# lueelu/DistributedFFT

Measured on AMD Instinct MI355X. Metric: GFlops/s forward 3D C2C (5 N log2 N), 512^3 fp64, higher is better.
Workload: dtype f64; 1 GPU; 512x512x512 C2C fp64 forward, slab decomposition over 1 GPU(s), fused pipeline, input resident in HBM; parallelism=slab1, exchange=none (P=1)

## Files before the change

### distributedfft_amd/csrc/dfft_core.cpp

```cpp
#include <cmath>
#include <map>
#include <mutex>

#include "dfft_plan_impl.h"
#include "dfft_r2r.h"
#include "dfft_real.h"
#include "dfft_real_cols.h"

namespace dfft {

static thread_local std::string g_last_error;
void set_error(const std::string& msg) { g_last_error = msg; }
int  fail(int code, const std::string& msg) {
    g_last_error = msg;
    trace_on_error(code, msg);
    return code;
}
const std::string& last_error() { return g_last_error; }

struct TwKey {
    int  dev, n, dtype;
    bool operator<(const TwKey& o) const {
        if (dev != o.dev) return dev < o.dev;
        if (n != o.n) return n < o.n;
// ... 129 lines not shown
    if (!valid_dtype(dtype) || kind < DFFT_R2R_DCT2 || kind > DFFT_R2R_DST3 || n < 1 || s < 1) return 0;
    return r2r_fused_env() && r2r_fused(n, s, dtype, kind, vec != 0);
}
int dfft_conv_fused_applies(int dtype, long long n0, long long rows, long long ncols, long long plane, long long pitch, int rot, const void* in,
                            const void* out) {
    if (!valid_dtype(dtype) || n0 < 1 || n0 > 4096 || rows < 1 || ncols < 1 || plane < 1 || pitch < 1 || rot < 0) return 0;
    ConvLaunch L;
    std::memset(&L, 0, sizeof(L));
    L.dtype = dtype;
    L.n0 = (int)n0;
    L.rows = rows;
    L.ncols = ncols;
    L.plane = plane;
    L.pitch = pitch;
    L.rot = rot;
    L.in = in;
    L.out = const_cast<void*>(out);
    return conv_fused_applies(L) ? 1 : 0;
}

int dfft_cols_extent_supported(long long n, long long width, int dtype, int pairs) {
    if (n < 1 || width < 1 || !valid_dtype(dtype) || length_kind(n) == 0 || length_kind(n) == 3) return 0;
    return cols_extent_ok(n, width, dtype, pairs != 0, pairs != 0) ? 1 : 0;
}
int dfft_fft1d_any_extent_supported(long long n, long long s, int dtype, int in16, int out16) {
    if (n < 1 || s < 1 || !valid_dtype(dtype) || length_kind(n) == 0) return 0;
    return any_extent_ok(n, s, dtype, in16 != 0, out16 != 0) ? 1 : 0;
}

static void scratch_tables(BluesteinTables* T, long long n, int dtype, int dir) {
    T->n = n;
    T->M = bluestein_padded_length(n);
    T->dtype = dtype;
    T->dir = dir;
}
unsigned long long dfft_fft1d_any_scratch_bytes(long long n, long long s, long long batch, int dtype) {
    const int kind = length_kind(n);
    if (!valid_dtype(dtype) || s < 1 || batch < 1 || kind < 2) return 0;
    if (kind == 2) return (unsigned long long)batch * n * s * elem_bytes(dtype);
    if (!bluestein_extent_ok(n, s, dtype)) return 0;
    BluesteinTables T;
    scratch_tables(&T, n, dtype, DFFT_FORWARD);
    return bluestein_scratch_bytes(T, s, batch, bluestein_fused_env());
}
unsigned long long dfft_rfft1d_strided_scratch_bytes(long long n, long long s, long long batch, int dtype) {
    const int kind = length_kind(n);
// ... 175 lines not shown
```

### distributedfft_amd/csrc/dfft_fft_impl.h

```cpp
#pragma once
#include <atomic>
#include <cstdio>
#include <cstdlib>
#include <mutex>
#include <type_traits>

#include "dfft_butterfly.h"
#include "dfft_kernels.h"

namespace dfft {

template <int N_, int E_, int... Rs> struct Plan {
    static constexpr int N = N_, E = E_, T = N_ / E_, S = sizeof...(Rs);
    static constexpr int R[sizeof...(Rs)] = {Rs...};
    static_assert((Rs * ... * 1) == N_, "radix product must equal N");
    static_assert(((E_ % Rs == 0) && ...), "every radix must divide E");
    static_assert(N_ % E_ == 0, "E must divide N");
};

struct TuneDefault {
    static constexpr bool TWPOW = true;
    static constexpr bool OSTAGE = false;
    static constexpr bool NTL = false;
    static constexpr bool NTS = false;
// ... 17 lines not shown
    static constexpr bool OSTAGE = true;
    static constexpr bool NTL = true;
    static constexpr bool NTS = true;
    static constexpr int MIN_WAVES = 0;
    static constexpr int CB_OVERRIDE = 0;
    static constexpr bool PLAIN = false;
    static constexpr bool PREFETCH = true;
    static constexpr bool FULL_PREFETCH = false;
    static constexpr bool PLAIN_IN = false;
    static constexpr bool EARLY_WAIT = false;
    static constexpr bool ROT = false;
    static constexpr int ROT_IN = 0, ROT_OUT = 0;
};
struct TuneTransposedStoreFull : TuneTransposedStore {
    static constexpr bool FULL_PREFETCH = true;
    static constexpr bool PLAIN_IN = true;
};
struct TuneTransposedStoreFullEarly : TuneTransposedStoreFull {
    static constexpr bool EARLY_WAIT = true;
};
struct TuneTransposedStoreEarly : TuneTransposedStore {
    static constexpr bool EARLY_WAIT = true;
};

struct TuneCols : TuneDefault {
    static constexpr bool PREFETCH = true;
};

template <class Base> struct Plain : Base {
    static constexpr bool PLAIN = true;
};

template <class Base> struct TransposedSide : Base {
    static constexpr bool NO_OWNED = true;
};
template <class T, class = void> struct tune_no_owned : std::false_type {};
template <class T> struct tune_no_owned<T, std::void_t<decltype(T::NO_OWNED)>> : std::bool_constant<T::NO_OWNED> {};

struct TuneStreamIn : TuneDefault {
    static constexpr bool NTL = true;
};
struct TuneColsStreamIn : TuneCols {
    static constexpr bool NTL = true;
};
struct TuneColsStreamOut : TuneCols {
    static constexpr bool NTS = true;
// ... 344 lines not shown
inline long long axis_max_offset(const AxisMap& m, int n) {
    long long mx = 0;
    const int nb = m.blk > 0 ? (n + m.blk - 1) / m.blk : 1;
    for (int ib = 0; ib < nb; ++ib) {
        const long long bt = m.sub > 1 ? (long long)(ib / m.sub) * m.blk_stride + (long long)(ib % m.sub) * m.sub_stride : (long long)ib * m.blk_stride;
        const int       cnt = (ib + 1) * m.blk <= n ? m.blk : n - ib * m.blk;
        const long long o = bt + (long long)(cnt - 1) * m.stride;
        if (o > mx) mx = o;
    }
    return mx;
}
inline bool tile_offsets_fit32(const FftLaunch& L) {
    auto fits = [&](const AxisMap& m) {
        const long long c = m.cstride < 0 ? -m.cstride : m.cstride;
        return axis_max_offset(m, L.n) + (kTileColsMax - 1) * c < (1ll << 32);
    };
    return fits(L.imap) && fits(L.omap);
}
template <class V, class P, int CB, int G, int DIR, bool GENERAL, class Tune>
__global__ void __attribute__((amdgpu_flat_work_group_size(1, KernelGeom<V, P, CB, G, Tune>::THREADS),
                               amdgpu_waves_per_eu(Tune::MIN_WAVES > 0 ? Tune::MIN_WAVES : 1)))
fft_tiles_kernel(const typename VecTraits<V>::G* in, typename VecTraits<V>::G* out,
                 const typename VecTraits<V>::W* __restrict__ tw, AxisMap imap, AxisMap omap, TileMap itile, TileMap otile,
                 unsigned ntiles, unsigned tiles_per_a, int ncols, unsigned a_first, double scale, RotMap rm) {
    using KG = KernelGeom<V, P, CB, G, Tune>;
    using VT = VecTraits<V>;
    using W = typename VT::W;
    using GV = typename VT::G;
    constexpr int E = P::E, T = P::T, GT = KG::GT, N = P::N, LANES = VT::LANES;
    extern __shared__ __attribute__((aligned(16))) char dfft_smem[];
    W* ldstw = reinterpret_cast<W*>(dfft_smem);
    V* lds = reinterpret_cast<V*>(dfft_smem + KG::TW_BYTES) + (threadIdx.x / GT) * KG::LDS_ELEMS;

    const int g = threadIdx.x / GT;
    const int tid = threadIdx.x - g * GT;
    const int c = tid % CB;
    const int j = tile_j<CB, KG::NW>(tid);

    constexpr int TWN = KG::TWMODE == TW_REG ? KG::TWN : 0;
    W twreg[TWN > 0 ? TWN : 1];
    const W* twr = stage_twiddles<V, P, DIR, KG, Tune::TWPOW>(twreg, ldstw, tw, j);
    constexpr bool TWPOW = Tune::TWPOW && KG::TWMODE == TW_REG;

    constexpr bool PLAIN = Tune::PLAIN && !GENERAL && !KG::OSTAGE && !Tune::ROT;
    constexpr bool PLAIN_IN = PLAIN || (Tune::PLAIN_IN && !GENERAL);
    constexpr int NREL = PLAIN ? 1 : E;
    constexpr int ON = N / LANES;
// ... 65 lines not shown
#pragma unroll
            for (int k = K0; k < K1; ++k) {
                long long off = PLAIN_IN ? (long long)(ir0 + (unsigned)k * istep) : (long long)irel[PLAIN_IN ? 0 : k];
                if (GENERAL) off += ((ilast >> k) & 1u) ? (long long)a * imap.last_delta : 0ll;
                if constexpr (Tune::ROT_IN == 2) off += (long long)(((cb0 + rj + k * rot_t) & rm.mask) - cb0);
                dst[k - K0] = VT::from_g(gload<Tune::NTL>(ip + off));
            }
        } else {
#pragma unroll
            for (int k = K0; k < K1; ++k) dst[k - K0] = VT::zero();
        }
    };
    auto load_tile = [&](unsigned t, V* dst) { load_part(t, dst, std::integral_constant<int, 0>{}, std::integral_constant<int, E>{}); };
    constexpr bool EARLY = Tune::EARLY_WAIT;
    constexpr bool P768 = P::N == 768 && E == 12 && sizeof(V) == 16;
    constexpr bool PREFETCH = Tune::PREFETCH && (E * (int)sizeof(V) / 4 <= kPrefetchMaxRegs || Tune::FULL_PREFETCH || P768) && KG::THREADS <= 512;
    constexpr int PF = PREFETCH ? E : (Tune::PREFETCH && KG::OSTAGE && E == 16 && sizeof(V) == 16 && KG::THREADS <= 512 && KG::PH == 1 ? E / 2 : 0);
    constexpr bool PARTIAL = PF > 0 && PF < E;
    using K0 = std::integral_constant<int, 0>;
    using KP = std::integral_constant<int, PF>;
    using KE = std::integral_constant<int, E>;
    V v[E];
    V vnext[PF > 0 ? PF : 1];
    if constexpr (PREFETCH) {
        if (blockIdx.x * G < ntiles) load_tile(blockIdx.x * G, v);
    } else if constexpr (PARTIAL) {
        if (blockIdx.x * G < ntiles) load_part(blockIdx.x * G, v, K0{}, KP{});
    }
    for (unsigned t0 = blockIdx.x * G; t0 < ntiles; t0 += tstep) {
        const unsigned tile = map_tile(t0 + g);
        bool valid = tile < ntiles;
        const unsigned al = tile / tiles_per_a;
        const unsigned b = tile - al * tiles_per_a;
        const unsigned a = al + a_first;
        if (GENERAL) valid = valid && ((int)(b * CB) + c < ncols);
        int ob0 = (int)(b * CB);
        if constexpr (Tune::ROT_OUT == 1) ob0 = (ob0 + rm.rot * (int)(a + (unsigned)rm.a0)) & rm.mask;
        GV* op = out + (long long)a * otile.a_stride + (long long)ob0 * otile.b_stride;

        if constexpr (PREFETCH) {
            if (t0 + tstep < ntiles) load_tile(t0 + tstep, vnext);
        } else if constexpr (PARTIAL) {
            load_part(t0, v + PF, KP{}, KE{});
            if (t0 + tstep < ntiles) load_part(t0 + tstep, vnext, K0{}, KP{});
        } else {
            load_tile(t0, v);
        }

        constexpr bool LOCALX = KG::LOCALX && !(GENERAL && P::N == 729 && CB > 1);
        run_stages<V, P, 0, DIR, CB, KG::PAD, KG::WAVE_LOCAL, KG::TWMODE, TWPOW, KG::PH, 1, KG::NW, LOCALX>(v, twr, lds, j, c);

        const typename real_of<W>::type sc = (typename real_of<W>::type)scale;

        if constexpr (KG::OSTAGE) {
            static_assert(!GENERAL || !KG::OSTAGE, "the staged store is a fast-path variant");
            constexpr int ROW = N + KG::OPAD;
            W* img = reinterpret_cast<W*>(lds);
            if constexpr (KG::PH == 1) {
                group_sync<KG::WAVE_LOCAL>();
#pragma unroll
                for (int k = 0; k < E; ++k)
#pragma unroll
                    for (int l = 0; l < LANES; ++l) img[(c * LANES + l) * ROW + j + T * k] = VT::lane(cscale(v[k], sc), l);
                group_sync<KG::WAVE_LOCAL>();
                if constexpr (EARLY && PF > 0) {
#pragma unroll
                    for (int k = 0; k < PF; ++k) pin_loaded(vnext[k]);
                }
                if (valid) {
#pragma unroll
                    for (int k = 0; k < E; ++k) {
                        const int lin = tid + GT * k;
                        const GV r = *reinterpret_cast<const GV*>(img + (lin / ON) * ROW + (lin % ON) * LANES);
                        gstore<Tune::NTS>(op + ostage_off(k), r);
                    }
                }
            } else {
                constexpr int CH = CB / KG::PH, EPH = E / KG::PH;
                const int     mine = c / CH, cl = c - mine * CH;
#pragma unroll
                for (int ph = 0; ph < KG::PH; ++ph) {
                    __syncthreads();
                    if (mine == ph) {
#pragma unroll
                        for (int k = 0; k < E; ++k)
#pragma unroll
                            for (int l = 0; l < LANES; ++l) img[(cl * LANES + l) * ROW + j + T * k] = VT::lane(cscale(v[k], sc), l);
// ... 7 lines not shown
                            gstore<Tune::NTS>(op + ostage_off(ph * EPH + k), r);
                        }
                    }
                }
            }
        } else if (valid) {
            if constexpr (EARLY && PF > 0) {
#pragma unroll
                for (int k = 0; k < PF; ++k) pin_loaded(vnext[k]);
            }
            unsigned or0 = orel[0];
            if constexpr (PLAIN) asm volatile("" : "+v"(or0));
#pragma unroll
            for (int k = 0; k < E; ++k) {
                long long off = PLAIN ? (long long)(or0 + (unsigned)k * ostep) : (long long)orel[PLAIN ? 0 : k];
                if (GENERAL) off += ((olast >> k) & 1u) ? (long long)a * omap.last_delta : 0ll;
                if constexpr (Tune::ROT_OUT == 2) off += (long long)(((ob0 + rot_j + k * rot_t) & rm.mask) - ob0);
                gstore<Tune::NTS>(op + off, VT::to_g(cscale(v[k], sc)));
            }
        }
        if constexpr (PF > 0) {
#pragma unroll
            for (int k = 0; k < PF; ++k) v[k] = vnext[k];
        }
    }
}

template <class V, class P, int CB> struct DualGeom {
    using W = typename VecTraits<V>::W;
    static constexpr int    LANES = VecTraits<V>::LANES, OPAD = LANES == 2 ? 2 : 1;
    static constexpr size_t BUDGET = 160 * 1024;
    static constexpr size_t TW_BYTES = ((size_t)P::N * sizeof(W) + 15) / 16 * 16;
    static constexpr bool   PADROW = (size_t)(P::N + OPAD) * CB * sizeof(V) + TW_BYTES <= BUDGET;
    static constexpr int    ROW = PADROW ? P::N + OPAD : P::N;
    static constexpr size_t LDS_BYTES = TW_BYTES + (size_t)ROW * CB * sizeof(V);
    static_assert(LDS_BYTES <= BUDGET, "dual tiles: tile + twiddle table must fit the workgroup's share of the CU's LDS");
};
template <class V, class P, int CB, int DIR, bool NT, bool ROT = false>
__global__ void __attribute__((amdgpu_flat_work_group_size(1, CB * P::T), amdgpu_waves_per_eu(1)))
fft_dual_tiles_kernel(const typename VecTraits<V>::G* in, typename VecTraits<V>::G* out, const typename VecTraits<V>::W* __restrict__ tw,
                      AxisMap imap, AxisMap omap, TileMap itile, TileMap otile, unsigned ntiles, unsigned tiles_per_a, unsigned a_first,
                      double scale, RotMap rm) {
    using VT = VecTraits<V>;
    using W = typename VT::W;
    using GV = typename VT::G;
    constexpr int E = P::E, T = P::T, GT = CB * T, N = P::N, LANES = VT::LANES;
// ... 399 lines not shown
    if (occ < 1) occ = 1;
    cache[dev].store(occ, std::memory_order_release);
    return occ;
}

inline long long persistent_grid(int cus, int blocks_per_cu, long long units, long long grid_limit = 0, int blocks_per_cu_limit = 0) {
    if (blocks_per_cu_limit > 0 && blocks_per_cu_limit < blocks_per_cu) blocks_per_cu = blocks_per_cu_limit;
    long long grid = (long long)cus * blocks_per_cu;
    if (grid_limit > 0 && grid > grid_limit) grid = grid_limit;
    return grid < units ? grid : units;
}

template <class V, class P, int CB, int G, int DIR, bool GENERAL, class Tune = TuneDefault>
hipError_t launch_variant(const FftLaunch& L, hipStream_t stream, int* blocks_per_cu_out = nullptr) {
    using KG = KernelGeom<V, P, CB, G, Tune>;
    auto kern = fft_tiles_kernel<V, P, CB, G, DIR, GENERAL, Tune>;
    static std::atomic<int> blocks_per_cu[kMaxDevices];
    hipError_t e;
    const int  bpc = resident_blocks_per_cu(reinterpret_cast<const void*>(kern), KG::THREADS, KG::LDS_BYTES, blocks_per_cu, &e);
    if (bpc == 0) return e;
    if (blocks_per_cu_out) *blocks_per_cu_out = bpc;
    const long long grid = persistent_grid(device_info().cus, bpc, (L.ntiles + G - 1) / G, L.grid_limit, L.blocks_per_cu_limit);
    if (grid < 1) return hipSuccess;
    (void)hipGetLastError();
    using GV = typename VecTraits<V>::G;
    hipLaunchKernelGGL(kern, dim3((unsigned)grid), dim3(KG::THREADS), KG::LDS_BYTES, stream, (const GV*)L.in, (GV*)L.out,
                       (const typename VecTraits<V>::W*)L.tw, L.imap, L.omap, L.itile, L.otile, (unsigned)L.ntiles,
                       (unsigned)L.tiles_per_a, L.ncols, (unsigned)L.a_first, L.scale == 0.0 ? 1.0 : L.scale, L.rot);
    e = hipGetLastError();
    if (e != hipSuccess) return launch_debug(e, "kernel launch", (int)KG::LDS_BYTES, KG::THREADS);
    return hipSuccess;
}

template <class V, class P, int CB, int DIR, bool NT, bool ROT = false> hipError_t launch_dual(const FftLaunch& L, hipStream_t stream) {
    using VT = VecTraits<V>;
    using W = typename VT::W;
    using GV = typename VT::G;
    constexpr size_t LDS_BYTES = DualGeom<V, P, CB>::LDS_BYTES;
    auto kern = fft_dual_tiles_kernel<V, P, CB, DIR, NT, ROT>;
    static std::atomic<int> attr_set[kMaxDevices];
    hipError_t e;
    if (resident_blocks_per_cu(reinterpret_cast<const void*>(kern), CB * P::T, LDS_BYTES, attr_set, &e, false) == 0) return e;
    const long long tiles_per_a = L.ncols / (2 * CB), ntiles = L.na * tiles_per_a;
    if (ntiles <= 0) return hipSuccess;
    if (ntiles >= (1ll << 31)) return hipErrorInvalidValue;
    const long long grid = persistent_grid(device_info().cus, 1, ntiles, L.grid_limit);
    (void)hipGetLastError();
    hipLaunchKernelGGL(kern, dim3((unsigned)grid), dim3(CB * P::T), LDS_BYTES, stream, (const GV*)L.in, (GV*)L.out, (const W*)L.tw, L.imap,
                       L.omap, L.itile, L.otile, (unsigned)ntiles, (unsigned)tiles_per_a, (unsigned)L.a_first, L.scale == 0.0 ? 1.0 : L.scale, L.rot);
    e = hipGetLastError();
    if (e != hipSuccess) return launch_debug(e, "kernel launch", (int)LDS_BYTES, CB * P::T);
    return hipSuccess;
}
// ... 139 lines not shown
        return launch_plan<V, P, PH, CBC / 2>(Lin, stream);
    } else if constexpr (CBC * P::T <= 1024) {
        if constexpr (CBO == 0 && can_tload<V, P>()) {
            if (tload_applies<V, P>(L)) {
                if (rot) return L.dir > 0 ? launch_tload<V, P, CBC, +1, true>(L, stream) : launch_tload<V, P, CBC, -1, true>(L, stream);
                return L.dir > 0 ? launch_tload<V, P, CBC, +1, false>(L, stream) : launch_tload<V, P, CBC, -1, false>(L, stream);
            }
        }
        if constexpr (VecTraits<V>::LANES == 2) {
            if (L.imap.nblk == 1 && L.imap.stride == 1 && L.imap.cstride != 1 && !(L.omap.nblk == 1 && L.omap.stride == 1 && L.omap.cstride != 1))
                return hipErrorInvalidValue;
        }
        using TT = TuneTransposedStore;
        using TTF = TuneTransposedStoreFull;
        constexpr bool can_stage = can_stage_store<V, P, CBO>();
        const bool staged = can_stage && !general && L.omap.nblk == 1 && L.omap.stride == 1 && L.omap.cstride != 1;
        constexpr bool can_full = can_stage && P::E == 16 && sizeof(V) == 16 && CBC * (int)sizeof(V) == 128 && CBC * P::T * GC <= 512;
        using TTFE = TuneTransposedStoreFullEarly;
        using TTE = TuneTransposedStoreEarly;
        const bool single_in = L.imap.nblk == 1 && L.imap.sub <= 1 && L.imap.last_delta == 0;
        const bool want_early = (L.hints & FFT_HINT_EARLY_WAIT) != 0;
        const int  full = (can_full && staged && L.dir > 0 && single_in && !(L.hints & FFT_HINT_HALF_PREFETCH)) ? (want_early ? 2 : 1) : 0;
        constexpr bool can_early = can_stage && P::N == 512 && sizeof(V) == 16;
        const bool early = can_early && staged && L.dir > 0 && want_early;
        constexpr bool can_dual = P::S > 1 && sizeof(V) == 16 && 2 * CBC * sizeof(V) == 128 && (P::N & (P::N - 1)) == 0 && (P::N / VecTraits<V>::LANES) % (CBC * P::T) == 0 &&
                                  (size_t)P::N * CBC * sizeof(V) + (size_t)P::N * sizeof(typename VecTraits<V>::W) <= 160 * 1024;
        if constexpr (!std::is_void<PH>::value && ((VecTraits<V>::LANES == 2 && P::N >= 2048) || (P::N == 1024 && VecTraits<V>::LANES == 1))) {
            static const bool x_dif2 = [] {
                const char* e = getenv("DFFT_X_DIF2");
                return !(e && *e == '0');
            }();
            constexpr int CBF = 128 / (int)sizeof(V);
            const bool    transposed = L.omap.nblk == 1 && L.omap.stride == 1 && L.omap.cstride != 1 && L.omap.last_delta == 0;
            constexpr bool want = P::N >= 2048 || VecTraits<V>::LANES == 1;
            if (x_dif2 && want && L.dir > 0 && !general && transposed && L.imap.cstride == 1 && L.itile.b_stride == 1 && L.imap.nblk == 1 && L.imap.sub <= 1 && L.ncols % CBF == 0 &&
                L.imap.last_delta == 0 && (axis_max_offset(L.imap, P::N / 2) + L.ncols) * (long long)sizeof(V) < (1ll << 32) && L.itile.b_stride == 1 &&
                (!rot || (L.rot.in_mode == 2 && L.rot.out_mode == 0))) {
                if (rot) return launch_dif2<V, PH, CBF, +1, true, true, false, false, 2, true>(L, stream);
                return launch_dif2<V, PH, CBF, +1, true, true, false, false, 0, true>(L, stream);
            }
        }
        if constexpr (can_dual) {
            static const bool no_dual = [] {
                const char* e = getenv("DFFT_NO_DUAL");
                return e && *e && *e != '0';
            }();
            const bool transposed = L.omap.nblk == 1 && L.omap.stride == 1 && L.omap.cstride != 1;
// ... 79 lines not shown
                return launch_variant<V, P, CBC, GC, -1, false, Plain<TuneCols>>(L, stream);
            }
        }
        const bool tr_side = !(L.imap.cstride == 1 && L.itile.b_stride == 1) || (!(L.omap.cstride == 1 && L.otile.b_stride == 1) && !(can_stage && staged));
        using TSCols = std::conditional_t<(KernelGeom<V, P, CBC, GC, TuneCols>::NW > 0), TransposedSide<TuneCols>, TuneCols>;
        using TSColsIn = std::conditional_t<(KernelGeom<V, P, CBC, GC, TuneColsStreamIn>::NW > 0), TransposedSide<TuneColsStreamIn>, TuneColsStreamIn>;
        using TSColsOut = std::conditional_t<(KernelGeom<V, P, CBC, GC, TuneColsStreamOut>::NW > 0), TransposedSide<TuneColsStreamOut>, TuneColsStreamOut>;
        if (tr_side) {
            if (L.dir > 0) {
                if (general) return launch_variant<V, P, CBC, GC, +1, true, TSCols>(L, stream);
                if (L.hints & FFT_HINT_STREAM_OUT) return launch_variant<V, P, CBC, GC, +1, false, TSColsOut>(L, stream);
                return launch_variant<V, P, CBC, GC, +1, false, TSCols>(L, stream);
            }
            if (general) return launch_variant<V, P, CBC, GC, -1, true, TSCols>(L, stream);
            if (L.hints & FFT_HINT_STREAM_IN) return launch_variant<V, P, CBC, GC, -1, false, TSColsIn>(L, stream);
            return launch_variant<V, P, CBC, GC, -1, false, TSCols>(L, stream);
        }
        if (L.dir > 0) {
            if (general) return launch_variant<V, P, CBC, GC, +1, true, TuneCols>(L, stream);
            if constexpr (can_full) {
                if (full == 2) return launch_variant<V, P, CBC, GC, +1, false, TTFE>(L, stream);
                if (full == 1) return launch_variant<V, P, CBC, GC, +1, false, TTF>(L, stream);
            }
            if constexpr (can_early)
                if (early) return launch_variant<V, P, CBC, GC, +1, false, TTE>(L, stream);
            if constexpr (can_stage)
                if (staged) return launch_variant<V, P, CBC, GC, +1, false, TT>(L, stream);
            if (L.hints & FFT_HINT_STREAM_OUT) return launch_variant<V, P, CBC, GC, +1, false, TuneColsStreamOut>(L, stream);
            return launch_variant<V, P, CBC, GC, +1, false, TuneCols>(L, stream);
        }
        if (general) return launch_variant<V, P, CBC, GC, -1, true, TuneCols>(L, stream);
        if constexpr (can_stage)
            if (staged) return launch_variant<V, P, CBC, GC, -1, false, TT>(L, stream);
        if (L.hints & FFT_HINT_STREAM_IN) return launch_variant<V, P, CBC, GC, -1, false, TuneColsStreamIn>(L, stream);
        return launch_variant<V, P, CBC, GC, -1, false, TuneCols>(L, stream);
    } else {
        return hipErrorInvalidValue;
    }
}

template <class P> bool make_pair_launch(const FftLaunch& L, FftLaunch& out) {
    static const bool disabled = [] {
        const char* e = getenv("DFFT_NO_PAIRS");
        return e && *e && *e != '0';
    }();
    if (disabled || !L.cols || L.dtype != F32 || L.ncols < 2 || (L.ncols & 1)) return false;
// ... 99 lines not shown
```

### distributedfft_amd/csrc/dfft_kernels.h

```cpp
#pragma once
#include <hip/hip_runtime.h>
#include <stdint.h>

namespace dfft {

enum DType { F64 = 0, F32 = 1 };

struct AxisMap {
    int       blk;
    int       nblk;
    long long blk_stride;
    long long stride;
    long long cstride;
    long long last_delta;
    int       sub;
    long long sub_stride;
};

struct TileMap {
    long long a_stride;
    long long b_stride;
};

struct RotMap {
// ... 3 lines not shown
    int a0;
};

struct FftLaunch {
    int         dtype;
    int         n;
    int         dir;
    int         cols;
    const void* in;
    void*       out;
    const void* tw;
    AxisMap     imap, omap;
    TileMap     itile, otile;
    long long   na;
    long long   ntiles;
    int         tiles_per_a;
    int         ncols;
    long long   a_first;
    int         hints;
    double      scale;
    int         blocks_per_cu_limit;
    RotMap      rot;
    int         grid_limit;
};
enum {
    FFT_HINT_STREAM_IN = 1,
    FFT_HINT_STREAM_OUT = 2,
    FFT_HINT_HALF_PREFETCH = 4,
    FFT_HINT_EARLY_WAIT = 8,
};

constexpr long long kTileColsMax = 64;
inline bool cols_offsets_fit32(long long n, long long stride_v) { return (n - 1) * stride_v + (kTileColsMax - 1) < (1ll << 32); }

bool fft_length_supported(int n);
bool fft_length_tuned(int n);
bool       generic_length_supported(int n);
hipError_t launch_generic(const struct FftLaunch& L, hipStream_t stream);
hipError_t launch_fft(const FftLaunch& L, hipStream_t stream);

hipError_t launch_pack(int dtype, int dir, const void* in, void* out, int xl, int n1, int n2, int yl,
                       int ylast, int P, hipStream_t stream);
hipError_t launch_transpose(int dtype, const void* in, void* out, long long rows, long long cols,
                            hipStream_t stream);
hipError_t launch_scale(int dtype, void* data, long long count, double s, hipStream_t stream);

}
```

### distributedfft_amd/csrc/dfft_plan.cpp

```cpp
#include <cstdio>
#include <numeric>

#include "dfft_plan_impl.h"

namespace dfft {

int fill_exchange(dfft_plan_s* p, ExchangeDesc& x, int direction) {
    const int       P = p->P, me = p->me;
    const long long n2 = p->N[2];
    x.dtype = p->dtype;
    x.direction = direction;
    x.P = P;
    x.me = me;
    x.scount.assign(P, 0);
    x.soffset.assign(P, 0);
    x.rcount.assign(P, 0);
    x.roffset.assign(P, 0);
    x.doffset.assign(P, 0);
    x.xsize.assign(P, 0);
    x.ysize.assign(P, 0);
    x.n2 = n2;
    for (int q = 0; q < P; ++q) {
        x.xsize[q] = p->sx.size(q);
        x.ysize[q] = p->sy.size(q);
// ... 114 lines not shown
        L.imap = L.omap = slab;
        L.itile = L.otile = slab_tile;
    } else if (p->direction == DFFT_FORWARD) {
        L.imap = slab;
        L.itile = slab_tile;
        L.omap = tr;
        L.otile = tr_tile;
    } else {
        L.imap = tr;
        L.itile = tr_tile;
        L.omap = slab;
        L.otile = slab_tile;
    }
    L.na = ys;
    L.scale = p->scale;
    L.ncols = (int)n2;
    if (p->rot_elems > 0 && p->exch && !keep_slab && !slab_lay) {
        L.rot.rot = p->rot_elems;
        L.rot.mask = (int)n2 - 1;
        (p->direction == DFFT_FORWARD ? L.rot.in_mode : L.rot.out_mode) = 2;
    }
    L.grid_limit = p->grid_x;
    L.hints |= p->x_hints;
    return check_launch(launch_fft(L, p->stream), "X pass");
}

int StageClock::begin() {
    if (sync) {
        DFFT_HIP_TRY(hipStreamSynchronize(p->stream));
        t = std::chrono::steady_clock::now();
    } else if (p->timed) {
        DFFT_HIP_TRY(hipEventRecord(p->ev[0], p->stream));
    }
    return DFFT_OK;
}
int StageClock::end_stage() {
    if (sync) {
        DFFT_HIP_TRY(hipStreamSynchronize(p->stream));
        auto now = std::chrono::steady_clock::now();
        p->host_t[idx] = std::chrono::duration<double>(now - t).count();
        t = now;
    } else if (p->timed) {
        DFFT_HIP_TRY(hipEventRecord(p->ev[idx + 1], p->stream));
    }
    ++idx;
    return DFFT_OK;
// ... 527 lines not shown
                if (getenv("DFFT_DEBUG")) fprintf(stderr, "[dfft] plan buffers: in %p out %p bufferDev1 %p work %p\n", in, out, p->buf1, p->wbuf);
            }
        }
    }
    {
        const char*     re = getenv("DFFT_ROT");
        const long long S = (long long)elem_bytes(dtype);
        const bool      possible = p->exch && !p->conv_no_rot && !(flags & (DFFT_PLAN_UNFUSED | DFFT_PLAN_NATURAL)) && !p->long_axis && n0 % total_devices == 0 &&
                              n1 % total_devices == 0 && (n2 & (n2 - 1)) == 0 && (n2 * S) % 128 == 0 && n2 * S >= 256 && n2 < (1ll << 30) &&
                              fft_length_tuned((int)n0) && fft_length_tuned((int)n1) && fft_length_tuned((int)n2);
        const long long ysub = p->ys / std::max(1, p->ycuts);
        const bool      pays = (ysub * n2 * S) % (128ll << 10) == 0;
        if (possible && !(re && *re == '0') && (pays || (re && *re == '1'))) {
            int         lines = (n0 >= 1024 && ysub * n2 * S >= (1ll << 20)) ? 2 : 3;
            const char* rl = getenv("DFFT_ROT_LINES");
            if (rl && atoi(rl) > 0) lines = atoi(rl);
            p->rot_elems = (int)(lines * 128 / S);
        }
    }
    {
        const char* xv = getenv("DFFT_X_VARIANT");
        if (xv && !strcmp(xv, "half")) p->x_hints = FFT_HINT_HALF_PREFETCH;
        else if (xv && (!strcmp(xv, "fullearly") || !strcmp(xv, "early"))) p->x_hints = FFT_HINT_EARLY_WAIT;
        const char* zl = getenv("DFFT_ZY_LAZY");
        p->zy_lazy = !(zl && *zl == '0');
        const char* rf = getenv("DFFT_ZY_INV_ROWS_FIRST");
        p->zy_inv_rows_first = !(rf && *rf == '0');
    }
    if (comm) {
        DFFT_TRY(place_recv_buffer(p));
        DFFT_TRY(comm_register(comm, global_idx, p->xd.recvbuf, p->device, &p->xd.slot));
    }
    {
        const char* oe = getenv("DFFT_T0_ONE_LAUNCH");
        const long long ysub = p->sy.blk / std::max(1, p->ycuts);
        const bool      single_ok = !p->exch && (!p->wbuf || p->wl.pitch == n2);
        const bool      multi_ok = p->exch && n0 % total_devices == 0 && n1 % total_devices == 0 && n1 >= 8 && ysub % zy_col_threads((int)n1, p->zy_lazy ? 1 : 0) == 0;
        const bool      parts_fwd = p->part_planes > 0 && direction == DFFT_FORWARD && p->zy_lazy;
        const bool      multi_on = (n1 == 512 && n2 == 512) || (n1 == 768 && n2 == 512 && (ysub % 64 == 0 || parts_fwd)) || (oe && !strcmp(oe, "all"));
        if (!(oe && *oe == '0') && (single_ok || (multi_ok && multi_on)) && !(flags & (DFFT_PLAN_UNFUSED | DFFT_PLAN_NATURAL)) && !p->long_axis &&
            zy_supported(dtype, (int)n1, (int)n2) && p->xs <= ZY_MAX_PLANES) {
            p->zy_eligible = true;
            if (hipMalloc((void**)&p->zy_ctl, sizeof(ZyCtl)) == hipSuccess && hipMemsetAsync(p->zy_ctl, 0, sizeof(ZyCtl), p->stream) == hipSuccess &&
                hipStreamSynchronize(p->stream) == hipSuccess && hipHostMalloc((void**)&p->zy_err, 128, hipHostMallocMapped) == hipSuccess) {
                *p->zy_err = 0u;
                p->zy_on = true;
// ... 147 lines not shown
            const void* src = (plan->flags & DFFT_PLAN_INPUT_FROM_IN) ? plan->in : plan->buf1;
            const bool  input_intact = !plan->exch && plan->wbuf && src != plan->buf2 && !(plan->flags & (DFFT_PLAN_UNFUSED | DFFT_PLAN_NATURAL)) &&
                                      !(plan->conv_half && plan->direction == DFFT_BACKWARD);
            if (!input_intact) return rc;
            if (getenv("DFFT_DEBUG")) fprintf(stderr, "[dfft] %s -- running the transform again on the two-launch stage\n", dfft_last_error());
            rc = run();
            if (rc) return rc;
        }
    }
    if (zrc0) return fail(zrc0, zmsg0);
    if (sync && plan->comm) {
        rc = comm_check(plan->comm);
        if (rc) return rc;
    }
    if ((exec_flags & DFFT_EXEC_PRINT) && plan->direction == DFFT_FORWARD) {
        double t[4];
        rc = dfft_stage_times(plan, t);
        if (rc) return rc;
        printf("t0: %lf, t1: %lf, t2: %lf, t3: %lf, total: %lf\n", t[0], t[1], t[2], t[3], t[0] + t[1] + t[2] + t[3]);
    }
    return DFFT_OK;
}

int dfft_plan_describe(dfft_plan_t plan, char* buf, int len) {
    if (!plan || !buf || len < 64) return fail(DFFT_EINVAL, "dfft_plan_describe: bad arguments");
    const dfft_plan_s* p = plan;
    if (p->conv) return conv_describe(p, buf, len);
    if (p->r2c) {
        snprintf(buf, (size_t)len, "pipeline=%s n2=%lld bins=%lld chunks=%lldx%lld intermediate_pitch=%lld", p->direction == DFFT_FORWARD ? "r2c" : "c2r",
                 p->n2r, p->N[2], p->chunk_planes > 0 ? (p->xs + p->chunk_planes - 1) / p->chunk_planes : 1ll, p->chunk_planes > 0 ? p->chunk_planes : p->xs,
                 p->cl.pitch);
        if (p->real_any) {
            const size_t used = strlen(buf);
            int          a = 0, b = 0;
            char         cf[96] = "";
            if (p->real_form == 3 && p->rtab)
                snprintf(cf, sizeof(cf), " complex_form=bluestein/M%lld/%s", p->rtab->M,
                         (p->n2r == 1 || (p->rfused && p->n2r <= kBluesteinFusedMaxLength)) ? "fused" : "multi-pass");
            else if (p->real_form == 3 && long_split(p->n2r, &a, &b))
                snprintf(cf, sizeof(cf), " complex_form=four-step/%dx%d", a, b);
            if (used + 1 < (size_t)len) snprintf(buf + used, (size_t)len - used, " real_form=%d%s", p->real_form, cf);
        }
        return DFFT_OK;
    }
    const bool         one = p->zy_on && !(p->flags & DFFT_PLAN_UNFUSED);
    const long long    cp = one ? zy_phase_planes(p, p->xs, p->exch && p->direction == DFFT_FORWARD) : (p->chunk_planes > 0 ? p->chunk_planes : p->xs);
    const long long    nch = cp > 0 ? (p->xs + cp - 1) / cp : 1;
    const bool         fused = !(p->flags & DFFT_PLAN_UNFUSED);
    snprintf(buf, (size_t)len,
             "pipeline=%s yz_stage=%s%s chunks=%lldx%lld handover=%s rotated_exchange_rows=%d overlap_parts=%lld ysub=%d parts_in_one_launch=%d tuned=%d x_variant=%s",
             (p->flags & DFFT_PLAN_NATURAL) ? "natural" : (fused ? "fused" : "unfused"),
             (p->zy_on && fused) ? "one-launch" : "two-launches-per-chunk", (p->zy_on && fused && p->zy_lazy) ? "-lazy" : "", nch, cp,
             (fused && p->wbuf && !p->exch) ? "padded-buffer" : "bufferDev1", p->rot_elems, p->part_planes, p->ycuts, (p->zy_on && fused && p->zy_part_done) ? 1 : 0, p->w_kept >= 0 ? 1 : 0,
             (p->x_hints & FFT_HINT_HALF_PREFETCH) ? "half-prefetch" : ((p->x_hints & FFT_HINT_EARLY_WAIT) ? "early-wait" : "default"));
    for (int a = 0; a < 3; ++a) {
        if (length_kind(p->N[a]) != 3 || p->bs.tables.empty()) continue;
        const size_t used = strlen(buf);
        if (used + 1 >= (size_t)len) break;
        const bool fused = p->N[a] == 1 || (p->bs.fused && p->N[a] <= kBluesteinFusedMaxLength);
        snprintf(buf + used, (size_t)len - used, " bluestein_axis%d=n%lld/M%lld/%s", a, p->N[a], bluestein_padded_length(p->N[a]),
                 fused ? "fused" : "multi-pass");
    }
    return DFFT_OK;
}

int dfft_plan_sync(dfft_plan_t plan) {
    if (!plan) return fail(DFFT_EINVAL, "dfft_plan_sync: null plan");
    if (plan->conv) return conv_sync(plan);
    if (plan->P > 1) trace("dfft_plan_sync enter", plan->direction, plan->flags);
    DFFT_HIP_TRY(hipStreamSynchronize(plan->stream));
    if (plan->P > 1) trace("dfft_plan_sync stream drained", plan->direction, plan->flags);
    {
        const int rc = zy_check(plan);
        if (rc) return rc;
    }
    if (plan->comm) return comm_check(plan->comm);
    return DFFT_OK;
// ... 61 lines not shown
    if (plan->stream2) hipStreamSynchronize(plan->stream2);
    const int zy_rc = zy_check(plan);
    if (plan->comm) {
        comm_unregister(plan->comm, plan->me, plan->xd2.slot);
        comm_unregister(plan->comm, plan->me, plan->xd.slot);
    }
    for (auto& e : plan->ev)
        if (e) hipEventDestroy(e);
    for (auto& e : plan->part_ev)
        if (e) hipEventDestroy(e);
    if (plan->join_ev) hipEventDestroy(plan->join_ev);
    for (auto& e : plan->y_ev)
        if (e) hipEventDestroy(e);
    if (plan->stream2) hipStreamDestroy(plan->stream2);
    if (plan->stream && !plan->borrowed) hipStreamDestroy(plan->stream);
    (void)comm_recv_free(plan->comm, plan->buf1);
    (void)comm_recv_free(plan->comm, plan->rbuf);
    if (plan->wbuf && !plan->borrowed) slab_free(plan->wbuf);
    if (plan->lbuf) hipFree(plan->lbuf);
    if (plan->bs.scratch) hipFree(plan->bs.scratch);
    if (plan->rscratch) hipFree(plan->rscratch);
    if (plan->cbuf && (!plan->borrowed || plan->own_cbuf)) hipFree(plan->cbuf);
    if (plan->zy_ctl) hipFree(plan->zy_ctl);
    if (plan->zy_part_done) hipFree(plan->zy_part_done);
    if (plan->zy_err) hipHostFree(plan->zy_err);
    delete plan;
    return zy_rc;
}

}
```

### distributedfft_amd/csrc/dfft_plan_impl.h

```cpp
#pragma once
#include <algorithm>
#include <chrono>
#include <cstdint>
#include <cstdlib>
#include <cstring>
#include <memory>
#include <string>
#include <vector>

#include "dfft_bluestein.h"
#include "dfft_conv.h"
#include "dfft_conv_multi.h"
#include "dfft_internal.h"
#include "dfft_long.h"
#include "dfft_zy.h"

#define DFFT_TRY(stmt)        \
    do {                      \
        int rc_ = (stmt);     \
        if (rc_) return rc_;  \
    } while (0)

namespace dfft {

// ... 78 lines not shown
    hipEvent_t              join_ev = nullptr;
    std::vector<hipEvent_t> part_ev;
    int                     ycuts = 1;
    std::vector<hipEvent_t> y_ev;
    void*                   wbuf = nullptr;
    dfft::SlabLayout        wl{0, 0};
    bool                    long_axis = false;
    void*                   lbuf = nullptr;
    dfft::PlanBluestein     bs;
    dfft::ZyCtl*            zy_ctl = nullptr;
    bool                    zy_eligible = false;
    unsigned*               zy_err = nullptr;
    unsigned                zy_spin_polls = 0;
    int                     zy_fault = 0;
    unsigned                zy_launches = 0;
    bool                    zy_on = false;
    unsigned                zy_ticket = 0;
    unsigned                zy_execs = 0, zy_cur = 0;
    unsigned*               zy_part_done = nullptr;
    unsigned                zy_sig_execs = 0;
    bool                    zy_lazy = false;
    bool                    zy_inv_rows_first = true;
    int                     x_hints = 0;
    int                     grid_x = 0, grid_y = 0, grid_z = 0;
    int                     rot_elems = 0;
    bool                    r2c = false;
    long long               n2r = 0;
    void*                   cbuf = nullptr;
    dfft::SlabLayout        cl{0, 0};
    bool                    real_any = false;
    int                     real_form = 1;
    dfft::BluesteinTablesPtr rtab;
    bool                    rfused = true;
    void*                   rscratch = nullptr;
    size_t                  rscratch_bytes = 0;
    struct ConvState*       conv = nullptr;
    bool                    conv_half = false, conv_no_rot = false, borrowed = false;
    bool                    own_cbuf = false;
    std::vector<float>      w_ms;
    int                     w_kept = -1;
    float                   w_final_ms = 0.f;
};

struct ConvState {
    dfft_plan_s *f = nullptr, *b = nullptr;
    void*        sbuf = nullptr;
// ... 96 lines not shown
```

Before: 9732 GFlops/s.

## Add atomic ticket-based dynamic tile scheduling to 512-point fp64 X pass

The 512-point fp64 forward X pass in the persistent tile kernel now hands out tiles through a global atomic ticket counter instead of a static blockIdx stride. Each workgroup draws two tickets ahead so the next-tile prefetch still works. The early-wait variant also becomes the default for this case. The goal is to balance load across CUs and cut tail imbalance, at the cost of an atomic per tile, an extra LDS broadcast, and a monotonically growing ticket base tracked on the host.

Result: faster. 10090 GFlops/s (median of 6 runs) (+3.7%).

```diff
diff --git a/distributedfft_amd/csrc/dfft_core.cpp b/distributedfft_amd/csrc/dfft_core.cpp
--- a/distributedfft_amd/csrc/dfft_core.cpp
+++ b/distributedfft_amd/csrc/dfft_core.cpp
@@ -175,6 +175,10 @@
 int dfft_cols_extent_supported(long long n, long long width, int dtype, int pairs) {
     if (n < 1 || width < 1 || !valid_dtype(dtype) || length_kind(n) == 0 || length_kind(n) == 3) return 0;
     return cols_extent_ok(n, width, dtype, pairs != 0, pairs != 0) ? 1 : 0;
+}
+unsigned dfft_x_ticket_base_after(unsigned base, long long ntiles, long long grid, long long launches) {
+    for (long long g = 0; g < launches; ++g) base += x_ticket_count((unsigned)ntiles, (unsigned)grid);
+    return base;
 }
 int dfft_fft1d_any_extent_supported(long long n, long long s, int dtype, int in16, int out16) {
     if (n < 1 || s < 1 || !valid_dtype(dtype) || length_kind(n) == 0) return 0;
diff --git a/distributedfft_amd/csrc/dfft_fft_impl.h b/distributedfft_amd/csrc/dfft_fft_impl.h
--- a/distributedfft_amd/csrc/dfft_fft_impl.h
+++ b/distributedfft_amd/csrc/dfft_fft_impl.h
@@ -63,6 +63,14 @@
 struct TuneTransposedStoreEarly : TuneTransposedStore {
     static constexpr bool EARLY_WAIT = true;
 };
+struct TuneTransposedStoreTicket : TuneTransposedStore {
+    static constexpr bool TICKET = true;
+};
+struct TuneTransposedStoreTicketEarly : TuneTransposedStoreEarly {
+    static constexpr bool TICKET = true;
+};
+template <class T, class = void> struct tune_ticket : std::false_type {};
+template <class T> struct tune_ticket<T, std::void_t<decltype(T::TICKET)>> : std::bool_constant<T::TICKET> {};
 
 struct TuneCols : TuneDefault {
     static constexpr bool PREFETCH = true;
@@ -453,7 +461,8 @@
                                amdgpu_waves_per_eu(Tune::MIN_WAVES > 0 ? Tune::MIN_WAVES : 1)))
 fft_tiles_kernel(const typename VecTraits<V>::G* in, typename VecTraits<V>::G* out,
                  const typename VecTraits<V>::W* __restrict__ tw, AxisMap imap, AxisMap omap, TileMap itile, TileMap otile,
-                 unsigned ntiles, unsigned tiles_per_a, int ncols, unsigned a_first, double scale, RotMap rm) {
+                 unsigned ntiles, unsigned tiles_per_a, int ncols, unsigned a_first, double scale, RotMap rm, unsigned* ticket_ctr,
+                 unsigned ticket_base) {
     using KG = KernelGeom<V, P, CB, G, Tune>;
     using VT = VecTraits<V>;
     using W = typename VT::W;
@@ -565,12 +574,35 @@
     using KE = std::integral_constant<int, E>;
     V v[E];
     V vnext[PF > 0 ? PF : 1];
-    if constexpr (PREFETCH) {
+    constexpr bool TICKET = tune_ticket<Tune>::value;
+    static_assert(!TICKET || (G == 1 && PREFETCH && KG::OSTAGE && KG::PH == 1 && !KG::WAVE_LOCAL && !GENERAL),
+                  "tickets: one block-wide tile per workgroup, whole-tile prefetch, one-phase staged store");
+    unsigned  first = 0, second = 0;
+    unsigned* ticket_word = nullptr;
+    auto take = [&]() -> unsigned {
+        return threadIdx.x == 0 ? __hip_atomic_fetch_add(ticket_ctr, 1u, __ATOMIC_RELAXED, __HIP_MEMORY_SCOPE_AGENT) - ticket_base : 0u;
+    };
+    if constexpr (TICKET) {
+        __shared__ unsigned ticket_lds[2];
+        ticket_word = ticket_lds;
+        const unsigned ta = take(), tb = take();
+        if (threadIdx.x == 0) {
+            ticket_lds[0] = ta;
+            ticket_lds[1] = tb;
+        }
+        __syncthreads();
+        first = __builtin_amdgcn_readfirstlane(ticket_lds[0]);
+        second = __builtin_amdgcn_readfirstlane(ticket_lds[1]);
+        if (first < ntiles) load_tile(first, v);
+    } else if constexpr (PREFETCH) {
         if (blockIdx.x * G < ntiles) load_tile(blockIdx.x * G, v);
     } else if constexpr (PARTIAL) {
         if (blockIdx.x * G < ntiles) load_part(blockIdx.x * G, v, K0{}, KP{});
     }
-    for (unsigned t0 = blockIdx.x * G; t0 < ntiles; t0 += tstep) {
+    for (unsigned t0 = TICKET ? first : blockIdx.x * G; t0 < ntiles; t0 = TICKET ? first : t0 + tstep) {
+        const unsigned tn = TICKET ? second : t0 + tstep;
+        unsigned       drawn = 0;
+        if constexpr (TICKET) drawn = take();
         const unsigned tile = map_tile(t0 + g);
         bool valid = tile < ntiles;
         const unsigned al = tile / tiles_per_a;
@@ -582,10 +614,10 @@
         GV* op = out + (long long)a * otile.a_stride + (long long)ob0 * otile.b_stride;
 
         if constexpr (PREFETCH) {
-            if (t0 + tstep < ntiles) load_tile(t0 + tstep, vnext);
+            if (tn < ntiles) load_tile(tn, vnext);
         } else if constexpr (PARTIAL) {
             load_part(t0, v + PF, KP{}, KE{});
-            if (t0 + tstep < ntiles) load_part(t0 + tstep, vnext, K0{}, KP{});
+            if (tn < ntiles) load_part(tn, vnext, K0{}, KP{});
         } else {
             load_tile(t0, v);
         }
@@ -605,7 +637,11 @@
                 for (int k = 0; k < E; ++k)
 #pragma unroll
                     for (int l = 0; l < LANES; ++l) img[(c * LANES + l) * ROW + j + T * k] = VT::lane(cscale(v[k], sc), l);
+                if constexpr (TICKET) {
+                    if (threadIdx.x == 0) ticket_word[0] = drawn;
+                }
                 group_sync<KG::WAVE_LOCAL>();
+                if constexpr (TICKET) drawn = __builtin_amdgcn_readfirstlane(ticket_word[0]);
                 if constexpr (EARLY && PF > 0) {
 #pragma unroll
                     for (int k = 0; k < PF; ++k) pin_loaded(vnext[k]);
@@ -659,6 +695,10 @@
         if constexpr (PF > 0) {
 #pragma unroll
             for (int k = 0; k < PF; ++k) v[k] = vnext[k];
+        }
+        if constexpr (TICKET) {
+            first = second;
+            second = drawn;
         }
     }
 }
@@ -1104,13 +1144,17 @@
     if (blocks_per_cu_out) *blocks_per_cu_out = bpc;
     const long long grid = persistent_grid(device_info().cus, bpc, (L.ntiles + G - 1) / G, L.grid_limit, L.blocks_per_cu_limit);
     if (grid < 1) return hipSuccess;
+    constexpr bool TICKET = tune_ticket<Tune>::value;
+    if (TICKET && (!L.x_ticket || !L.x_ticket_base)) return hipErrorInvalidValue;
     (void)hipGetLastError();
     using GV = typename VecTraits<V>::G;
     hipLaunchKernelGGL(kern, dim3((unsigned)grid), dim3(KG::THREADS), KG::LDS_BYTES, stream, (const GV*)L.in, (GV*)L.out,
                        (const typename VecTraits<V>::W*)L.tw, L.imap, L.omap, L.itile, L.otile, (unsigned)L.ntiles,
-                       (unsigned)L.tiles_per_a, L.ncols, (unsigned)L.a_first, L.scale == 0.0 ? 1.0 : L.scale, L.rot);
+                       (unsigned)L.tiles_per_a, L.ncols, (unsigned)L.a_first, L.scale == 0.0 ? 1.0 : L.scale, L.rot,
+                       TICKET ? L.x_ticket : nullptr, TICKET ? *L.x_ticket_base : 0u);
     e = hipGetLastError();
     if (e != hipSuccess) return launch_debug(e, "kernel launch", (int)KG::LDS_BYTES, KG::THREADS);
+    if (TICKET) *L.x_ticket_base += x_ticket_count((unsigned)L.ntiles, (unsigned)grid);
     return hipSuccess;
 }
 
@@ -1296,7 +1340,12 @@
         const bool want_early = (L.hints & FFT_HINT_EARLY_WAIT) != 0;
         const int  full = (can_full && staged && L.dir > 0 && single_in && !(L.hints & FFT_HINT_HALF_PREFETCH)) ? (want_early ? 2 : 1) : 0;
         constexpr bool can_early = can_stage && P::N == 512 && sizeof(V) == 16;
-        const bool early = can_early && staged && L.dir > 0 && want_early;
+        constexpr bool x512_f64 = can_early && VecTraits<V>::LANES == 1 && CBO == 0;
+        using TTK = TuneTransposedStoreTicket;
+        using TTKE = TuneTransposedStoreTicketEarly;
+        const bool plan_x = x512_f64 && staged && L.dir > 0 && !rot && L.x_ticket && L.x_ticket_base;
+        const bool early = can_early && staged && L.dir > 0 && (want_early || (plan_x && !(L.hints & FFT_HINT_LATE_WAIT)));
+        const bool ticket = plan_x && !(L.hints & FFT_HINT_STATIC_TILES);
         constexpr bool can_dual = P::S > 1 && sizeof(V) == 16 && 2 * CBC * sizeof(V) == 128 && (P::N & (P::N - 1)) == 0 && (P::N / VecTraits<V>::LANES) % (CBC * P::T) == 0 &&
                                   (size_t)P::N * CBC * sizeof(V) + (size_t)P::N * sizeof(typename VecTraits<V>::W) <= 160 * 1024;
         if constexpr (!std::is_void<PH>::value && ((VecTraits<V>::LANES == 2 && P::N >= 2048) || (P::N == 1024 && VecTraits<V>::LANES == 1))) {
@@ -1422,6 +1471,10 @@
                 if (full == 2) return launch_variant<V, P, CBC, GC, +1, false, TTFE>(L, stream);
                 if (full == 1) return launch_variant<V, P, CBC, GC, +1, false, TTF>(L, stream);
             }
+            if constexpr (x512_f64) {
+                if (plan_x && L.x_form) *L.x_form = X_FORM_512_F64 | (early ? X_FORM_EARLY : 0) | (ticket ? X_FORM_TICKET : 0);
+                if (ticket) return early ? launch_variant<V, P, CBC, GC, +1, false, TTKE>(L, stream) : launch_variant<V, P, CBC, GC, +1, false, TTK>(L, stream);
+            }
             if constexpr (can_early)
                 if (early) return launch_variant<V, P, CBC, GC, +1, false, TTE>(L, stream);
             if constexpr (can_stage)
diff --git a/distributedfft_amd/csrc/dfft_kernels.h b/distributedfft_amd/csrc/dfft_kernels.h
--- a/distributedfft_amd/csrc/dfft_kernels.h
+++ b/distributedfft_amd/csrc/dfft_kernels.h
@@ -49,12 +49,19 @@
     int         blocks_per_cu_limit;
     RotMap      rot;
     int         grid_limit;
+    unsigned*   x_ticket;
+    unsigned*   x_ticket_base;
+    int*        x_form;
 };
+enum { X_FORM_512_F64 = 1, X_FORM_EARLY = 2, X_FORM_TICKET = 4 };
+inline unsigned x_ticket_count(unsigned ntiles, unsigned grid) { return ntiles + 2u * grid; }
 enum {
     FFT_HINT_STREAM_IN = 1,
     FFT_HINT_STREAM_OUT = 2,
     FFT_HINT_HALF_PREFETCH = 4,
     FFT_HINT_EARLY_WAIT = 8,
+    FFT_HINT_LATE_WAIT = 16,
+    FFT_HINT_STATIC_TILES = 32,
 };
 
 constexpr long long kTileColsMax = 64;
diff --git a/distributedfft_amd/csrc/dfft_plan.cpp b/distributedfft_amd/csrc/dfft_plan.cpp
--- a/distributedfft_amd/csrc/dfft_plan.cpp
+++ b/distributedfft_amd/csrc/dfft_plan.cpp
@@ -160,6 +160,14 @@
     }
     L.grid_limit = p->grid_x;
     L.hints |= p->x_hints;
+    if (p->x_ticket_ctr && ys_part <= 0 && !keep_slab) {
+        L.x_ticket = p->x_ticket_ctr;
+        L.x_ticket_base = &p->x_ticket;
+    }
+    if (ys_part <= 0) {
+        p->x_form = 0;
+        L.x_form = &p->x_form;
+    }
     return check_launch(launch_fft(L, p->stream), "X pass");
 }
 
@@ -733,6 +741,15 @@
         const char* xv = getenv("DFFT_X_VARIANT");
         if (xv && !strcmp(xv, "half")) p->x_hints = FFT_HINT_HALF_PREFETCH;
         else if (xv && (!strcmp(xv, "fullearly") || !strcmp(xv, "early"))) p->x_hints = FFT_HINT_EARLY_WAIT;
+        else if (xv && !strcmp(xv, "static")) p->x_hints = FFT_HINT_STATIC_TILES;
+        else if (xv && !strcmp(xv, "late")) p->x_hints = FFT_HINT_LATE_WAIT;
+        else if (xv && !strcmp(xv, "static-late")) p->x_hints = FFT_HINT_STATIC_TILES | FFT_HINT_LATE_WAIT;
+        if (dtype == F64 && n0 == 512 && direction == DFFT_FORWARD && n2 % 8 == 0 && !p->exch && !(flags & DFFT_PLAN_NATURAL) && !p->long_axis) {
+            if (hipMalloc((void**)&p->x_ticket_ctr, sizeof(unsigned)) != hipSuccess || hipMemsetAsync(p->x_ticket_ctr, 0, sizeof(unsigned), p->stream) != hipSuccess ||
+                hipStreamSynchronize(p->stream) != hipSuccess)
+                return fail(DFFT_EHIP, "dfft_plan_create: no ticket counter for the X pass");
+            p->x_form = X_FORM_512_F64 | ((p->x_hints & FFT_HINT_LATE_WAIT) ? 0 : X_FORM_EARLY) | ((p->x_hints & FFT_HINT_STATIC_TILES) ? 0 : X_FORM_TICKET);
+        }
         const char* zl = getenv("DFFT_ZY_LAZY");
         p->zy_lazy = !(zl && *zl == '0');
         const char* rf = getenv("DFFT_ZY_INV_ROWS_FIRST");
@@ -926,6 +943,15 @@
     return DFFT_OK;
 }
 
+static const char* x_variant_name(const dfft_plan_s* p) {
+    if (p->x_form & X_FORM_512_F64) {
+        const bool early = (p->x_form & X_FORM_EARLY) != 0;
+        if (p->x_form & X_FORM_TICKET) return early ? "ticket-early-wait" : "ticket-late-wait";
+        return early ? "static-early-wait" : "static-late-wait";
+    }
+    return (p->x_hints & FFT_HINT_HALF_PREFETCH) ? "half-prefetch" : ((p->x_hints & FFT_HINT_EARLY_WAIT) ? "early-wait" : "default");
+}
+
 int dfft_plan_describe(dfft_plan_t plan, char* buf, int len) {
     if (!plan || !buf || len < 64) return fail(DFFT_EINVAL, "dfft_plan_describe: bad arguments");
     const dfft_plan_s* p = plan;
@@ -956,7 +982,7 @@
              (p->flags & DFFT_PLAN_NATURAL) ? "natural" : (fused ? "fused" : "unfused"),
              (p->zy_on && fused) ? "one-launch" : "two-launches-per-chunk", (p->zy_on && fused && p->zy_lazy) ? "-lazy" : "", nch, cp,
              (fused && p->wbuf && !p->exch) ? "padded-buffer" : "bufferDev1", p->rot_elems, p->part_planes, p->ycuts, (p->zy_on && fused && p->zy_part_done) ? 1 : 0, p->w_kept >= 0 ? 1 : 0,
-             (p->x_hints & FFT_HINT_HALF_PREFETCH) ? "half-prefetch" : ((p->x_hints & FFT_HINT_EARLY_WAIT) ? "early-wait" : "default"));
+             x_variant_name(p));
     for (int a = 0; a < 3; ++a) {
         if (length_kind(p->N[a]) != 3 || p->bs.tables.empty()) continue;
         const size_t used = strlen(buf);
@@ -1064,6 +1090,7 @@
     if (plan->rscratch) hipFree(plan->rscratch);
     if (plan->cbuf && (!plan->borrowed || plan->own_cbuf)) hipFree(plan->cbuf);
     if (plan->zy_ctl) hipFree(plan->zy_ctl);
+    if (plan->x_ticket_ctr) hipFree(plan->x_ticket_ctr);
     if (plan->zy_part_done) hipFree(plan->zy_part_done);
     if (plan->zy_err) hipHostFree(plan->zy_err);
     delete plan;
diff --git a/distributedfft_amd/csrc/dfft_plan_impl.h b/distributedfft_amd/csrc/dfft_plan_impl.h
--- a/distributedfft_amd/csrc/dfft_plan_impl.h
+++ b/distributedfft_amd/csrc/dfft_plan_impl.h
@@ -124,6 +124,9 @@
     bool                    zy_lazy = false;
     bool                    zy_inv_rows_first = true;
     int                     x_hints = 0;
+    unsigned*               x_ticket_ctr = nullptr;
+    unsigned                x_ticket = 0;
+    int                     x_form = 0;
     int                     grid_x = 0, grid_y = 0, grid_z = 0;
     int                     rot_elems = 0;
     bool                    r2c = false;
```
